# Potato256/my-mitsuba

Measured on AMD Instinct MI355X. Metric: Msamples/sec at 1280x720x256spp, 1/2/4/8 MI355X; per-pixel L1 vs CPU ref, higher is better.
Workload: dtype f32; 1 GPU; C3 bunny x15, 1,041,765 triangles, roughconductor Cu GGX 0.2, 15 instances flattened to world-space triangles; resolution=1280x720, spp=256, max_depth=8, parallelism=film tiles round-robin over 1 GPU(s), kd_build=host, kd_refs=4723933, kd_stop_prims=4

## Files before the change

include/mtsg.h:

```cpp
#ifndef MTSG_H
#define MTSG_H

#include <stdint.h>
#include <stddef.h>

#ifdef __cplusplus
extern "C" {
#endif

#define MTSG_ABI_VERSION 8

enum {
    MTSG_OK             = 0,
    MTSG_ERR_INVALID    = -1,
    MTSG_ERR_DEVICE     = -2,
    MTSG_ERR_OOM        = -3,
    MTSG_ERR_CANCELLED  = -4,
    MTSG_ERR_NODEVICE   = -5,
    MTSG_ERR_TRAVERSAL  = -6
};


typedef struct mtsg_kdnode {
    uint32_t combined;
// ... 349 lines not shown

int  mtsg_device_alloc(mtsg_scene *scene, size_t bytes, void **out);
int  mtsg_device_free(mtsg_scene *scene, void *ptr);
int  mtsg_device_memset(mtsg_scene *scene, void *ptr, size_t bytes);
int  mtsg_device_to_host(mtsg_scene *scene, void *dst, const void *src, size_t bytes);

void mtsg_cancel(mtsg_scene *scene);

void mtsg_cancel_clear(mtsg_scene *scene);

typedef void (*mtsg_tile_fn)(void *user, int32_t key, int32_t x, int32_t y, int32_t w, int32_t h);
int  mtsg_set_tile_callback(mtsg_scene *scene, mtsg_tile_fn fn, void *user);

int  mtsg_set_flags(mtsg_scene *scene, uint32_t flags);
int  mtsg_get_stats(mtsg_scene *scene, mtsg_stats *out);
int  mtsg_debug_wavetimes(mtsg_scene *scene, uint64_t *out, uint32_t max_launches, uint32_t *waves);
int  mtsg_debug_stragglers(mtsg_scene *scene, float *out, uint32_t max_rays);

int  mtsg_set_batch_paths(mtsg_scene *scene, uint32_t paths);

#define MTSG_DEFAULT_FINISH_PATHS 524288u
int  mtsg_set_finish_paths(mtsg_scene *scene, uint32_t paths);

#define MTSG_RECT_SETUP_CAP 2u
enum {
    MTSG_OPT_TRACE_REFILL = 1,
    MTSG_OPT_FINISH_SHADE_MIN = 2,
    MTSG_OPT_LANES = 3,
    MTSG_OPT_STAGGER = 4,
    MTSG_OPT_SHADE_GENERIC = 5,
    MTSG_OPT_RAY_ORDER = 6,
    MTSG_OPT_CAMERA_DIFFS = 7,
    MTSG_OPT_RECT_SETUP = 8,
    MTSG_OPT_RAY_PRESETUP = 9
};
int  mtsg_set_option(mtsg_scene *scene, int32_t key, int64_t value);

enum { MTSG_EMITTER_SET_AREA = 0, MTSG_EMITTER_SET_ENVMAP = 1, MTSG_EMITTER_SET_ALL = 2 };
int  mtsg_scene_kernel_sets(mtsg_scene *scene, int32_t *material_set, int32_t *emitter_set);

typedef struct mtsg_test_knobs {
    int32_t stack_cap, restart_guard, restart_limit, limit_shadow_only;
    int32_t no_instance_prefilter;
} mtsg_test_knobs;
int  mtsg_set_test_knobs(mtsg_scene *scene, const mtsg_test_knobs *knobs);

int  mtsg_env_eval(mtsg_scene *scene, uint32_t n, const float *dirs, const float *rx, const float *ry, float *out);

int  mtsg_tex_eval(mtsg_scene *scene, int tex, uint32_t n, const float *uv, const float *duv, float *out);

enum { MTSG_BSDF_QUERY_SAMPLE = 0, MTSG_BSDF_QUERY_EVAL = 1 };
enum { MTSG_BSDF_QUERY_OK = 1, MTSG_BSDF_QUERY_DELTA = 2, MTSG_BSDF_QUERY_NULL = 4 };
int  mtsg_bsdf_query(mtsg_scene *scene, int32_t bsdf, int32_t mode, uint32_t n, const float *in, const float *alb, float *out,
                     uint32_t *flags);

int  mtsg_om_query(mtsg_scene *scene, uint32_t n, const float *dirs, const float *o1, const float *o2, int32_t *ids,
                   int32_t *vis);
// ... 103 lines not shown
```

my-mitsuba_amd/csrc/kernels.h:

```cpp
#pragma once
#include <hip/hip_runtime.h>

#include <stdint.h>

#include "../../include/mtsg.h"
#include "device_math.h"
#include "envmap.h"
#include "sampler.h"

namespace mtsg {

struct DevCamera;
struct DevScene {
    const uint4 *__restrict__ blocks;
    uint2 root2;
    const float4 *__restrict__ triL;
    const float4 *__restrict__ vpos;
    const float4 *__restrict__ vnrm;
    const uint4 *__restrict__ tidx;
    const float4 *__restrict__ shrec;
    const mtsg_rect *__restrict__ rects;
    const float4 *__restrict__ rectM;
    uint32_t n_rect;
    const float4 *__restrict__ rectSh;
// ... 115 lines not shown
template <int SMP> void launch_finish_ext2(const ShadeLaunch &a);
#define MTSG_DECLARE_LAUNCHERS(SMP) \
    template <> void launch_shade_smp<SMP>(const ShadeLaunch &a); \
    template <> void launch_finish_smp<SMP>(const ShadeLaunch &a); \
    template <> void launch_shade_ext2<SMP>(const ShadeLaunch &a); \
    template <> void launch_finish_ext2<SMP>(const ShadeLaunch &a);
MTSG_DECLARE_LAUNCHERS(MTSG_SAMPLER_INDEPENDENT)
MTSG_DECLARE_LAUNCHERS(MTSG_SAMPLER_HALTON)
MTSG_DECLARE_LAUNCHERS(MTSG_SAMPLER_HAMMERSLEY)
MTSG_DECLARE_LAUNCHERS(MTSG_SAMPLER_LDSAMPLER)
MTSG_DECLARE_LAUNCHERS(MTSG_SAMPLER_SOBOL)
int finish_blocks_per_cu(bool mats);
struct FlatTraceLaunch {
    dim3 grid, tieGrid;
    hipStream_t stream;
    const DevScene *S;
    const DevPaths *P;
    int cIn, sIn;
    uint32_t n;
    unsigned long long *wt;
    bool count, knobs, refill32, tie;
    bool rectSetup;
    bool pre = false;
};
void launch_trace_flat(const FlatTraceLaunch &a);
int trace_flat_blocks_per_cu();

struct DevAov {
    int m;
    int pathChild;
    int nf;
    int kind[MTSG_MAX_SUBINTEGRATORS];
    int child[MTSG_MAX_SUBINTEGRATORS];
    float undef[MTSG_MAX_SUBINTEGRATORS][3];
    float w2c[16];
    const mtsg_aov_bsdf *bsdfs;
    const mtsg_aov_shape *shapes;
    const uint32_t *elems;
    float *planes;
    size_t cap;
};
struct FieldsLaunch {
    hipStream_t stream;
    const DevScene *S;
    const DevCamera *C;
    const DevIntegrator *I;
// ... 3769 lines not shown
```

my-mitsuba_amd/csrc/mtsg.hip:

```cpp
#include <hip/hip_runtime.h>

#include <algorithm>
#include <atomic>
#include <cstdio>
#include <cstdlib>
#include <cstring>
#include <mutex>
#include <string>
#include <unordered_map>
#include <vector>
#include <chrono>
#include <functional>

#include "../../include/mtsg.h"
#include "device_math.h"
#include "envmap.h"
#include "sampler.h"

#include "kernels.h"
#include "render_plan.h"

#ifndef MTSG_RAY_PRESETUP
#define MTSG_RAY_PRESETUP 0
#endif

static_assert(PLAN_TILE == TILE, "render_plan.h plans in tiles of kernels.h's edge");

namespace {

thread_local std::string g_err;

#define HIP_TRY(expr)                                                                  \
    do {                                                                               \
        hipError_t _e = (expr);                                                        \
        if (_e != hipSuccess) {                                                        \
            g_err = std::string(#expr) + ": " + hipGetErrorString(_e);                 \
            return _e == hipErrorOutOfMemory ? MTSG_ERR_OOM : MTSG_ERR_DEVICE;         \
        }                                                                              \
    } while (0)

template <class T>
int upload(const T *src, size_t n, T **dst) {
    *dst = nullptr;
    if (n == 0) return MTSG_OK;
    HIP_TRY(hipMalloc((void **)dst, n * sizeof(T)));
    HIP_TRY(hipMemcpy(*dst, src, n * sizeof(T), hipMemcpyHostToDevice));
// ... 33 lines not shown
    int lanesAlloc = 0;
    hipStream_t lstream[MTSG_MAX_LANES] = {};
    std::vector<int32_t> tileKeys;
    int32_t *tileKeysDev = nullptr;
    size_t tileKeysCap = 0;
    DevPaths LP[MTSG_MAX_LANES]{};
    std::vector<void *> batchAllocs;
    uint32_t *hostCnt = nullptr;
    int cuCount = 0;
    int traceGrid = 0, shadeGrid = 0, traceGridInst = 0, finishGrid = 0, finishGridMats = 0;
    uint32_t finishPaths = 0;
    uint32_t finishShadeMin = 16;
    uint32_t flags = 0;
    int samplerType = MTSG_SAMPLER_INDEPENDENT, samplerDim = 4;
    int qmcInv[2][3] = {{0, 0, 0}, {0, 0, 0}};
    int traceMode = 0;
    bool texDiffs = false, hasEnvmap = false, storeCamDiffs = false;
    int rayOrder = 0;
    float *dumpL = nullptr;
    std::atomic<int> cancel{0};
    bool knobs = false;
    bool rectSetupOpt = true, rectSetupOk = false;
    bool rayPresetupOpt = MTSG_RAY_PRESETUP != 0;
    mtsg_stats stats{};
    std::vector<hipEvent_t> evPool;
    size_t evUsed = 0;
    std::vector<std::pair<int, size_t>> timed;
    std::vector<unsigned long long> stragglers;
    unsigned long long *waveTimes = nullptr;
    uint32_t wtLaunches = 0;
    bool extBsdfs = false;
    bool ext2 = false;
    int mats = MATS_ALL;
    bool shadeGeneric = false;
    int emitterSet = EM_AREA;
    uint32_t nTextures = 0;
    const uint32_t *sobolM = nullptr;
    const uint64_t *sobolVdc = nullptr, *sobolVdcInv = nullptr;
    uint64_t sobolScramble = 0;
    bool aovOn = false;
    DevAov aov{};
    std::vector<void *> aovAllocs;
    float *fieldPlanes = nullptr;
    size_t fieldCap = 0;
    int fieldCount = 0;
    uint32_t nShapes = 0;
// ... 115 lines not shown
    return s->evPool[s->evUsed++];
}

template <class F>
void timed_launch(mtsg_scene *s, int kind, hipStream_t st, F f) {
    if (!(s->flags & MTSG_FLAG_TIMING)) { f(); return; }
    size_t i0 = s->evUsed;
    hipEventRecord(next_event(s), st);
    f();
    hipEventRecord(next_event(s), st);
    s->timed.emplace_back(kind, i0);
}

template <bool COUNT>
void launch_trace_c(mtsg_scene *s, const DevPaths &P, int cIn, int sIn, uint32_t n, hipStream_t st, bool pre) {
    dim3 g(s->traceGrid), blk(TRACE_BLOCK);
    unsigned long long *wt = nullptr;
    if ((s->flags & MTSG_FLAG_WAVETIME) && s->waveTimes && s->wtLaunches < WT_MAX_LAUNCHES && !s->ds.inst)
        wt = s->waveTimes + (size_t)WT_WORDS * s->traceGrid * s->wtLaunches++;
    const dim3 tg(std::max<unsigned>(1u, (unsigned)s->traceGrid / 4u));
    if (!s->ds.inst) {
        FlatTraceLaunch a{g, tg, st, &s->ds, &P, cIn, sIn, n, wt, COUNT, s->knobs, s->traceMode == 1,
                          MTSG_MAILBOX && cIn != -2 && !TIE_INLINE, s->rectSetupOpt && s->rectSetupOk, pre};
        launch_trace_flat(a);
        return;
    }
    if (s->knobs && !COUNT)
        hipLaunchKernelGGL((k_trace_s<false, MTSG_INST_MIN_IDLE, true, true>), dim3(s->traceGridInst), blk, 0, st, s->ds, P, cIn, sIn, n, wt);
    else hipLaunchKernelGGL((k_trace_s<COUNT, MTSG_INST_MIN_IDLE, true>), dim3(s->traceGridInst), blk, 0, st, s->ds, P, cIn, sIn, n, wt);
    if (MTSG_MAILBOX && cIn != -2) hipLaunchKernelGGL(k_tie_i, tg, blk, 0, st, s->ds, P);
}
void launch_trace(mtsg_scene *s, bool count, const DevPaths &P, int cIn, int sIn, uint32_t n, hipStream_t st, bool pre = false) {
    if (count) launch_trace_c<true>(s, P, cIn, sIn, n, st, pre);
    else launch_trace_c<false>(s, P, cIn, sIn, n, st, pre);
}
bool presetup_applies(const mtsg_scene *s) {
    return s->rayPresetupOpt && s->rectSetupOpt && s->rectSetupOk && !s->ds.inst && !s->knobs;
}

ShadeLaunch shade_args(mtsg_scene *s, const DevIntegrator &I, const DevBatch &B, const DevPaths &P, int b, int qin, hipStream_t st,
                       dim3 grid, dim3 block) {
    ShadeLaunch a;
    a.grid = grid;
    a.block = block;
    a.stream = st;
    a.S = &s->ds;
// ... 746 lines not shown
        if (ti.x >= d->n_vertices || ti.y >= d->n_vertices || ti.z >= d->n_vertices || ti.w >= d->n_shapes) {
            g_err = "triangle index out of range";
            return fail(MTSG_ERR_INVALID);
        }
        const float *P = d->vtx_pos, *N = d->vtx_nrm;
        float f[24];
        for (int k = 0; k < 3; ++k) {
            f[k] = P[3 * ti.x + k]; f[3 + k] = P[3 * ti.y + k]; f[6 + k] = P[3 * ti.z + k];
            f[9 + k] = N[3 * ti.x + k]; f[12 + k] = N[3 * ti.y + k]; f[15 + k] = N[3 * ti.z + k];
            f[18 + k] = d->tri_dpdu[3 * t + k];
        }
        const mtsg_shape &sh = d->shapes[ti.w];
        uint32_t u[3] = {ti.w, (uint32_t)sh.bsdf | (sh.face_normals ? 0x80000000u : 0u), (uint32_t)sh.emitter};
        memcpy(f + 21, u, sizeof(u));
        memcpy(&shrec[6 * (size_t)t], f, sizeof(f));
    }
    int rc;
    DevScene &ds = s->ds;
    auto up = [&](auto *src, size_t n, auto **dst) {
        int r = upload(src, n, dst);
        if (r == MTSG_OK && *dst) s->allocs.push_back((void *)*dst);
        return r;
    };
    std::vector<uint4> pairs;
    std::vector<float4> triL;
    pairs.reserve(d->n_nodes / 2 + 1);
    triL.reserve((size_t)d->n_indices * 3);
    bool layoutOk = true;
    const mtsg_kdnode *tNodes = d->nodes;
    const uint32_t *tIdx = d->indices;
    uint32_t tNodeCount = d->n_nodes, tIdxCount = d->n_indices;
    std::function<uint2(uint32_t, int)> convert = [&](uint32_t ni, int depth) -> uint2 {
        if (depth > 64 || ni >= tNodeCount) { layoutOk = false; return make_uint2(0x80000000u, 0u); }
        const mtsg_kdnode &N = tNodes[ni];
        if (N.combined & 0x80000000u) {
            const uint32_t start = (uint32_t)(triL.size() / 3);
            for (uint32_t e = N.combined & 0x7FFFFFFFu; e < N.data; ++e) {
                const uint32_t p = e < tIdxCount ? tIdx[e] : 0xFFFFFFFFu;
                if (p >= d->n_prims) { layoutOk = false; break; }
                mtsg_triaccel ta = d->triaccel[p];
                if (ta.k == MTSG_TRIACCEL_SHAPE && ta.shape_index < d->n_shapes &&
                    d->shapes[ta.shape_index].type == MTSG_SHAPE_INSTANCE) {
                    if (ta.prim_index >= d->n_instances) { layoutOk = false; break; }
                    ta.k = KINST;
                    const mtsg_instance &I = d->instances[ta.prim_index];
                    if (I.group >= d->n_groups) { layoutOk = false; break; }
                    const mtsg_group &G = d->groups[I.group];
                    double lo[3] = {INFINITY, INFINITY, INFINITY}, hi[3] = {-INFINITY, -INFINITY, -INFINITY};
                    for (int c = 0; c < 8; ++c) {
                        const double q[3] = {(c & 1) ? G.aabb_max[0] : G.aabb_min[0], (c & 2) ? G.aabb_max[1] : G.aabb_min[1],
                                             (c & 4) ? G.aabb_max[2] : G.aabb_min[2]};
                        for (int a = 0; a < 3; ++a) {
                            const float *W = I.to_world + 4 * a;
                            const double w = (double)W[0] * q[0] + (double)W[1] * q[1] + (double)W[2] * q[2] + (double)W[3];
                            lo[a] = std::min(lo[a], w);
                            hi[a] = std::max(hi[a], w);
                        }
                    }
                    double ext = 0, mag = 0;
                    for (int a = 0; a < 3; ++a) {
                        ext = std::max(ext, hi[a] - lo[a]);
                        mag = std::max(mag, std::max(std::fabs(lo[a]), std::fabs(hi[a])));
                    }
                    const double m = 1e-4 * (ext + mag) + 1e-30;
                    float bmin[3], bmax[3];
                    for (int a = 0; a < 3; ++a) {
                        bmin[a] = std::nextafter((float)(lo[a] - m), -INFINITY);
                        bmax[a] = std::nextafter((float)(hi[a] + m), INFINITY);
                    }
                    if (!std::isfinite(bmin[0] + bmin[1] + bmin[2] + bmax[0] + bmax[1] + bmax[2])) {
                        for (int a = 0; a < 3; ++a) { bmin[a] = -INFINITY; bmax[a] = INFINITY; }
                    }
                    ta.n_u = bmin[0]; ta.n_v = bmin[1]; ta.n_d = bmin[2];
                    ta.a_u = bmax[0]; ta.a_v = bmax[1]; ta.b_nu = bmax[2];
                }
                ta.shape_index = p;
                const float4 *t = (const float4 *)&ta;
                triL.push_back(t[0]); triL.push_back(t[1]); triL.push_back(t[2]);
            }
            return make_uint2(0x80000000u | start, (uint32_t)(triL.size() / 3));
        }
        const uint32_t left = ni + ((N.combined & ~(3u | 0x40000000u)) >> 2);
        const uint32_t pi = (uint32_t)pairs.size();
        pairs.push_back(make_uint4(0, 0, 0, 0));
        const uint2 L = convert(left, depth + 1);
        const uint2 R = convert(left + 1, depth + 1);
        pairs[pi] = make_uint4(L.x, L.y, R.x, R.y);
        return make_uint2((N.combined & 3u) | (pi << 2), N.data);
    };
    const uint2 root = convert(0, 0);
    std::vector<uint2> groupRoots(d->n_groups);
    if (d->n_instances && (!d->instances || !d->groups || !d->group_nodes || !d->group_indices)) layoutOk = false;
    for (uint32_t g = 0; g < d->n_groups && layoutOk; ++g) {
        const mtsg_group &G = d->groups[g];
        if ((uint64_t)G.node_offset + G.n_nodes > d->n_group_nodes || (uint64_t)G.index_offset + G.n_indices > d->n_group_indices ||
            G.n_nodes == 0) { layoutOk = false; break; }
        tNodes = d->group_nodes + G.node_offset;
        tIdx = d->group_indices + G.index_offset;
        tNodeCount = G.n_nodes;
        tIdxCount = G.n_indices;
        groupRoots[g] = convert(0, 0);
    }
    for (uint32_t i = 0; i < d->n_instances && layoutOk; ++i)
        if (d->instances[i].group >= d->n_groups) layoutOk = false;
    if (!layoutOk || pairs.size() >= (1u << 29) || triL.size() / 3 >= (1u << 30)) {
        g_err = "malformed or oversized kd-tree";
        return fail(MTSG_ERR_INVALID);
    }
    std::vector<uint4> blocks;
    blocks.reserve(pairs.size() * 2 + 8);
    std::unordered_map<uint32_t, uint32_t> preBlock;
    auto reserveBlock = [&](uint32_t pair) {
        preBlock[pair] = (uint32_t)(blocks.size() / 4);
        blocks.resize(blocks.size() + 4, make_uint4(0, 0, 0, 0));
    };
    if (!(root.x & 0x80000000u)) {
        reserveBlock(root.x >> 2);
        const uint4 pr = pairs[root.x >> 2];
        for (const uint2 c : {make_uint2(pr.x, pr.y), make_uint2(pr.z, pr.w)}) {
            if (c.x & 0x80000000u) continue;
            const uint4 gp = pairs[c.x >> 2];
            for (const uint2 g : {make_uint2(gp.x, gp.y), make_uint2(gp.z, gp.w)})
                if (!(g.x & 0x80000000u)) reserveBlock(g.x >> 2);
        }
    }
    std::function<uint2(uint2, bool, uint32_t)> conv2 = [&](uint2 w, bool root, uint32_t slot) -> uint2 {
        if (w.x & 0x80000000u) return w;
        const uint4 pr = pairs[w.x >> 2];
        const uint2 L = make_uint2(pr.x, pr.y), R = make_uint2(pr.z, pr.w);
        if (root) {
            uint32_t b;
            const auto pre = preBlock.find(w.x >> 2);
            if (pre != preBlock.end()) {
                b = pre->second;
            } else {
                b = (uint32_t)(blocks.size() / 4);
                blocks.resize(blocks.size() + 4, make_uint4(0, 0, 0, 0));
            }
            const uint2 nL = conv2(L, false, 4 * b + 1);
            const uint2 nR = conv2(R, false, 4 * b + 2);
            blocks[4 * b] = make_uint4(nL.x, nL.y, nR.x, nR.y);
            return make_uint2((w.x & 3u) | (b << 3), w.y);
        }
        const uint2 nL = conv2(L, true, 0), nR = conv2(R, true, 0);
        blocks[slot] = make_uint4(nL.x, nL.y, nR.x, nR.y);
        return make_uint2((w.x & 3u) | 4u | (slot << 3), w.y);
    };
    const uint2 root2 = conv2(root, true, 0);
    for (auto &gr : groupRoots) gr = conv2(gr, true, 0);
    blocks.resize(blocks.size() + 4, make_uint4(0, 0, 0, 0));
    if (blocks.size() < 20) blocks.resize(20, make_uint4(0, 0, 0, 0));
    if (blocks.size() >= (1u << 29)) { g_err = "kd-tree too large for the two-level layout"; return fail(MTSG_ERR_INVALID); }
    if (triL.empty()) triL.resize(3, make_float4(0, 0, 0, 0));
    uint4 *dblocks; float4 *dtriL; float4 *dvpos, *dvnrm, *dshrec; uint4 *dtidx;
    mtsg_rect *rects; mtsg_shape *shapes; mtsg_bsdf *bsdfs; mtsg_emitter *emitters; float *ecdf, *etcdf;
    if ((rc = up(triL.data(), triL.size(), &dtriL)) ||
        (rc = up(blocks.data(), blocks.size(), &dblocks)) ||
        (rc = up(vpos.data(), vpos.size(), &dvpos)) || (rc = up(vnrm.data(), vnrm.size(), &dvnrm)) ||
        (rc = up(tidx.data(), tidx.size(), &dtidx)) ||
        (rc = up(shrec.data(), shrec.size(), &dshrec)) ||
        (rc = up(d->rects, d->n_rects, &rects)) || (rc = up(d->shapes, d->n_shapes, &shapes)) ||
        (rc = up(d->bsdfs, d->n_bsdfs, &bsdfs)) || (rc = up(d->emitters, d->n_emitters, &emitters)) ||
        (rc = up(d->emitter_cdf, d->n_emitters + 1, &ecdf)) ||
        (rc = up(d->emitter_tri_cdf, d->n_emitter_tri_cdf, &etcdf)))
        return fail(rc);
    ds.blocks = dblocks; ds.root2 = root2;
    ds.triL = dtriL; ds.vpos = dvpos; ds.vnrm = dvnrm;
    int constantEmitter = -1;
    {
        std::vector<float4> rm((size_t)3 * std::max<uint32_t>(d->n_rects, 1u), make_float4(0, 0, 0, 0));
        for (uint32_t i = 0; i < d->n_rects; ++i)
            for (int k = 0; k < 3; ++k) {
                const float *m = d->rects[i].to_object + 4 * k;
                rm[3 * i + k] = make_float4(m[0], m[1], m[2], m[3]);
            }
        if (d->n_bsdfs >= 0xFFFFu || d->n_emitters >= 0xFFFEu) { g_err = "too many BSDFs or emitters"; return fail(MTSG_ERR_INVALID); }
        std::vector<float4> rs((size_t)2 * std::max<uint32_t>(d->n_rects, 1u), make_float4(0, 0, 0, 0));
        for (uint32_t i = 0; i < d->n_rects; ++i) {
            const mtsg_rect &R = d->rects[i];
            if (R.shape_index >= d->n_shapes) { g_err = "rectangle with an invalid shape index"; return fail(MTSG_ERR_INVALID); }
            const mtsg_shape &sh = d->shapes[R.shape_index];
            uint32_t be = ((uint32_t)sh.bsdf & 0xFFFFu) | (uint32_t)(sh.emitter + 1) << 16, si = R.shape_index;
            float bef, sif;
            memcpy(&bef, &be, 4);
            memcpy(&sif, &si, 4);
            rs[2 * i] = make_float4(R.frame_n[0], R.frame_n[1], R.frame_n[2], sif);
            rs[2 * i + 1] = make_float4(R.dpdu[0], R.dpdu[1], R.dpdu[2], bef);
        }
        std::vector<float4> er((size_t)4 * std::max<uint32_t>(d->n_emitters, 1u), make_float4(0, 0, 0, 0));
// ... 57 lines not shown
            memcpy(&er[4 * e + 3].w, &type, 4);
        }
        float4 *drm, *drs, *der;
        if ((rc = up(rm.data(), rm.size(), &drm)) || (rc = up(rs.data(), rs.size(), &drs)) || (rc = up(er.data(), er.size(), &der)))
            return fail(rc);
        ds.rectM = drm;
        ds.rectSh = drs;
        ds.emitRect = der;
    }
    ds.tidx = dtidx; ds.shrec = dshrec; ds.rects = rects; ds.shapes = shapes; ds.bsdfs = bsdfs;
    ds.emitters = emitters; ds.emitter_cdf = ecdf; ds.emitter_tri_cdf = etcdf;
    ds.inst = nullptr;
    if (d->n_instances) {
        std::vector<float4> in((size_t)8 * d->n_instances);
        for (uint32_t i = 0; i < d->n_instances; ++i) {
            const mtsg_instance &I = d->instances[i];
            const mtsg_group &G = d->groups[I.group];
            const float *L = I.to_local, *W = I.to_world;
            float4 *o = &in[8 * (size_t)i];
            for (int r = 0; r < 3; ++r) {
                o[r] = make_float4(L[4 * r], L[4 * r + 1], L[4 * r + 2], L[4 * r + 3]);
                o[3 + r] = make_float4(W[4 * r], W[4 * r + 1], W[4 * r + 2], W[4 * r + 3]);
            }
            const uint2 gr = groupRoots[I.group];
            float r0, r1;
            memcpy(&r0, &gr.x, 4);
            memcpy(&r1, &gr.y, 4);
            o[6] = make_float4(G.aabb_min[0], G.aabb_min[1], G.aabb_min[2], r0);
            o[7] = make_float4(G.aabb_max[0], G.aabb_max[1], G.aabb_max[2], r1);
        }
        float4 *dinst;
        if ((rc = up(in.data(), in.size(), &dinst))) return fail(rc);
        ds.inst = dinst;
    }
    ds.capFlat = SHORT_STACK;
    ds.capGrp = INNER_STACK;
    ds.capTop = OUTER_STACK;
    ds.rstGuard = RST_GUARD;
    ds.rstMax = RST_MAX;
    ds.rstMaxC = RST_MAX;
    ds.instPrefilter = 1;
    s->knobs = false;
    ds.instKeyStride = (uint64_t)d->n_prims * ((uint64_t)d->n_instances + 1) <= 0xFFFFFFFFull ? d->n_prims : 0x9E3779B1u;
    ds.has_env = d->has_envmap ? 1 : constantEmitter >= 0 ? 2 * (constantEmitter + 1) : 0;
    if (s->emitterSet != EM_ALL) s->emitterSet = d->has_envmap ? EM_ENV : EM_AREA;
    s->mats = 0;
    for (uint32_t i = 0; i < d->n_bsdfs; ++i) {
// ... 86 lines not shown
            tt[3 * t + 2] = make_float4(dv[2], 0.f, 0.f, 0.f);
        }
        float4 *dttex;
        if ((rc = up(tt.data(), tt.size(), &dttex))) return fail(rc);
        ds.ttex = dttex;
    }
    s->nShapes = d->n_shapes;
    s->bsdfTexture.resize(d->n_bsdfs);
    for (uint32_t i = 0; i < d->n_bsdfs; ++i) s->bsdfTexture[i] = d->bsdfs[i].texture;
    s->texDiffs = texDiffs;
    s->hasEnvmap = d->has_envmap != 0;
    ds.om = nullptr; ds.om_bits = nullptr;
    if (d->om) {
        if (!d->om_bits) { g_err = "occupancy maps without their bits"; return fail(MTSG_ERR_INVALID); }
        mtsg_om *dom; uint32_t *dbits;
        if ((rc = up(d->om, 1, &dom)) ||
            (rc = up(d->om_bits, (size_t)MTSG_OM_COUNT * MTSG_OM_SIZE * MTSG_OM_SIZE * (MTSG_OM_SIZE / 32), &dbits)))
            return fail(rc);
        ds.om = dom; ds.om_bits = dbits;
    }
    ds.n_emitters = d->n_emitters;
    ds.n_tri = d->n_triangles;
    ds.n_rect = d->n_rects;
    s->rectSetupOk = MTSG_RECT_SETUP && d->n_rects <= RECT_SETUP_CAP;
    for (uint32_t r = 0; r < d->n_rects && s->rectSetupOk; ++r) {
        const mtsg_triaccel &ta = d->triaccel[d->n_triangles + r];
        s->rectSetupOk = ta.k == MTSG_TRIACCEL_SHAPE && ta.prim_index == r && ta.shape_index < d->n_shapes &&
                         d->shapes[ta.shape_index].type == MTSG_SHAPE_RECT;
    }
    ds.n_bsdfs = d->n_bsdfs;
    for (int k = 0; k < 3; ++k) { ds.bmin[k] = d->aabb_min[k]; ds.bmax[k] = d->aabb_max[k]; }
    DevCamera &c = s->cam;
    const mtsg_camera &hc = d->camera;
    memcpy(c.s2c, hc.sample_to_camera, sizeof(c.s2c));
    memcpy(c.c2w, hc.camera_to_world, sizeof(c.c2w));
    c.near_clip = hc.near_clip; c.far_clip = hc.far_clip; c.inv_res_x = hc.inv_res_x; c.inv_res_y = hc.inv_res_y;
    c.film_w = hc.film_w; c.film_h = hc.film_h;
    c.filter_radius = hc.filter_radius; c.filter_scale = hc.filter_scale; c.border = hc.border;
    c.has_alpha = hc.has_alpha;
    memcpy(c.filter_values, hc.filter_values, sizeof(c.filter_values));
    memcpy(c.dx, hc.dx, sizeof(c.dx));
    memcpy(c.dy, hc.dy, sizeof(c.dy));
    c.crop_w = hc.crop_w; c.crop_h = hc.crop_h;
    c.lens = hc.sensor_type == MTSG_SENSOR_THINLENS ? 1 : 0;
    c.aperture_radius = hc.aperture_radius; c.focus_distance = hc.focus_distance;
    ds.camO[0] = c.c2w[3]; ds.camO[1] = c.c2w[7]; ds.camO[2] = c.c2w[11];
    ds.camNear = c.near_clip; ds.camFar = c.far_clip;
    ds.camCompact = (ds.inst || c.lens) ? 0 : 1;
    c.compact = ds.camCompact;
    camera_diff_mode(s);
    {
        DevCamera *dc;
// ... 140 lines not shown
            if (value < 0 || value > 16) { g_err = "MTSG_OPT_STAGGER: 0..16 bounces"; return MTSG_ERR_INVALID; }
            s->stagger = (int)value;
            return MTSG_OK;
        case MTSG_OPT_SHADE_GENERIC:
            s->shadeGeneric = value != 0;
            return MTSG_OK;
        case MTSG_OPT_RAY_ORDER:
            if (value < 0 || value > 1) { g_err = "MTSG_OPT_RAY_ORDER: 0 (append order) or 1 (direction-sorted windows)"; return MTSG_ERR_INVALID; }
            s->rayOrder = (int)value;
            return MTSG_OK;
        case MTSG_OPT_CAMERA_DIFFS:
            if (value < 0 || value > 1) { g_err = "MTSG_OPT_CAMERA_DIFFS: 0 (recomputed on a miss) or 1 (stored)"; return MTSG_ERR_INVALID; }
            s->storeCamDiffs = value != 0;
            camera_diff_mode(s);
            return MTSG_OK;
        case MTSG_OPT_RECT_SETUP:
            if (value < 0 || value > 1) { g_err = "MTSG_OPT_RECT_SETUP: 0 (rectangles tested in the leaves) or 1 (at ray setup)"; return MTSG_ERR_INVALID; }
            s->rectSetupOpt = value != 0;
            return MTSG_OK;
        case MTSG_OPT_RAY_PRESETUP:
            if (value < 0 || value > 1) { g_err = "MTSG_OPT_RAY_PRESETUP: 0 (rectangles tested in the traversal's refill) or 1 (where the rays are made)"; return MTSG_ERR_INVALID; }
            s->rayPresetupOpt = value != 0;
            return MTSG_OK;
        default:
            g_err = "unknown option key " + std::to_string(key);
            return MTSG_ERR_INVALID;
    }
}

int mtsg_set_flags(mtsg_scene *s, uint32_t flags) {
    if (!s) return MTSG_ERR_INVALID;
    s->flags = flags;
    return MTSG_OK;
}

int mtsg_get_stats(mtsg_scene *s, mtsg_stats *out) {
    if (!s || !out) return MTSG_ERR_INVALID;
    *out = s->stats;
    return MTSG_OK;
}

int mtsg_debug_wavetimes(mtsg_scene *s, uint64_t *out, uint32_t max_launches, uint32_t *waves) {
    if (!s || !waves || (!out && max_launches)) return MTSG_ERR_INVALID;
    *waves = (uint32_t)s->traceGrid;
    const uint32_t n = std::min(max_launches, s->wtLaunches);
    if (n && s->waveTimes &&
// ... 649 lines not shown
```

my-mitsuba_amd/csrc/trace_flat.hip:

```cpp
#pragma clang diagnostic ignored "-Wunused-function"
#ifndef MTSG_STACK_LANE
#define MTSG_STACK_LANE 1
#endif
#include "kernels.h"

#if MTSG_FLAT_REGS
namespace {
#define FLAT_TRACE_KERNEL(MIN_IDLE, KNOBS)                                                                               \
    template <>                                                                                                          \
    __global__ void FLAT_TRACE_ATTR k_trace_s<false, MIN_IDLE, false, KNOBS>(DevScene S, DevPaths P, int cIn, int sIn,   \
                                                                             uint32_t nIdentity, unsigned long long *wt) { \
        trace_s_body<false, MIN_IDLE, false, KNOBS>(S, P, cIn, sIn, nIdentity, wt);                                      \
    }
FLAT_TRACE_KERNEL(16, false)
FLAT_TRACE_KERNEL(32, false)
FLAT_TRACE_KERNEL(16, true)
#undef FLAT_TRACE_KERNEL
}
#endif

namespace mtsg {

template <bool COUNT>
static void launch_flat(const FlatTraceLaunch &a) {
    const dim3 blk(TRACE_BLOCK);
    if (a.pre && a.rectSetup && !a.knobs) {
        if (a.refill32) hipLaunchKernelGGL((k_trace_s_pre<COUNT, 32>), a.grid, blk, 0, a.stream, *a.S, *a.P, a.cIn, a.sIn, a.n, a.wt);
        else hipLaunchKernelGGL((k_trace_s_pre<COUNT, 16>), a.grid, blk, 0, a.stream, *a.S, *a.P, a.cIn, a.sIn, a.n, a.wt);
    } else if (a.knobs && !COUNT) hipLaunchKernelGGL((k_trace_s<false, 16, false, true>), a.grid, blk, 0, a.stream, *a.S, *a.P, a.cIn, a.sIn, a.n, a.wt);
    else if (!a.rectSetup && a.refill32) hipLaunchKernelGGL((k_trace_s_leaf<COUNT, 32>), a.grid, blk, 0, a.stream, *a.S, *a.P, a.cIn, a.sIn, a.n, a.wt);
    else if (!a.rectSetup) hipLaunchKernelGGL((k_trace_s_leaf<COUNT, 16>), a.grid, blk, 0, a.stream, *a.S, *a.P, a.cIn, a.sIn, a.n, a.wt);
    else if (a.refill32) hipLaunchKernelGGL((k_trace_s<COUNT, 32>), a.grid, blk, 0, a.stream, *a.S, *a.P, a.cIn, a.sIn, a.n, a.wt);
    else hipLaunchKernelGGL((k_trace_s<COUNT, 16>), a.grid, blk, 0, a.stream, *a.S, *a.P, a.cIn, a.sIn, a.n, a.wt);
    if (a.tie) {
        if (a.knobs) hipLaunchKernelGGL((k_tie<true>), a.tieGrid, blk, 0, a.stream, *a.S, *a.P);
        else hipLaunchKernelGGL((k_tie<false>), a.tieGrid, blk, 0, a.stream, *a.S, *a.P);
    }
}

void launch_trace_flat(const FlatTraceLaunch &a) {
    if (a.count) launch_flat<true>(a);
    else launch_flat<false>(a);
}

int trace_flat_blocks_per_cu() {
    int perCU = 0;
    if (hipOccupancyMaxActiveBlocksPerMultiprocessor(&perCU, (const void *)k_trace_s<false, 16>, TRACE_BLOCK, 0) != hipSuccess) return 0;
    return perCU;
}
// ... 3 lines not shown
```

my-mitsuba_amd/mtsg.py:

```python
from __future__ import annotations

import ctypes as C
import os

import numpy as np

PKG_DIR = os.path.dirname(os.path.abspath(__file__))
REPO_DIR = os.path.dirname(PKG_DIR)

MTSG_OK = 0
MTSH_INSTANCING_FLATTEN = 0
MTSH_INSTANCING_TWO_LEVEL = 1
MTSG_FLAG_TIMING = 1
MTSG_FLAG_COUNT = 2
MTSG_FLAG_WAVETIME = 4
MTSG_OPT_TRACE_REFILL = 1
MTSG_OPT_FINISH_SHADE_MIN = 2
MTSG_OPT_LANES = 3
MTSG_OPT_STAGGER = 4
MTSG_OPT_SHADE_GENERIC = 5
MTSG_OPT_RAY_ORDER = 6
MTSG_OPT_CAMERA_DIFFS = 7
MTSG_OPT_RECT_SETUP = 8
MTSG_OPT_RAY_PRESETUP = 9
MTSG_RECT_SETUP_CAP = 2
MTSG_INTEGRATOR_PATH = 0
MTSG_INTEGRATOR_PATH2_OM = 1
MTSG_INTEGRATOR_DIRECT = 2
MTSG_INTEGRATOR_AO = 3
MTSG_EMITTER_AREA, MTSG_EMITTER_ENVMAP, MTSG_EMITTER_POINT, MTSG_EMITTER_SPOT = 1, 2, 3, 4
MTSG_EMITTER_DIRECTIONAL, MTSG_EMITTER_CONSTANT = 5, 6


class RenderParams(C.Structure):
    _fields_ = [
        ("max_depth", C.c_int32), ("rr_depth", C.c_int32),
        ("strict_normals", C.c_int32), ("hide_emitters", C.c_int32),
        ("spp", C.c_uint32), ("seed", C.c_uint32),
        ("tile_x", C.c_int32), ("tile_y", C.c_int32),
        ("tile_w", C.c_int32), ("tile_h", C.c_int32),
        ("tile_stride", C.c_int32), ("tile_offset", C.c_int32),
        ("integrator", C.c_int32), ("om_strategy", C.c_int32), ("om_mis", C.c_int32), ("om_jitter", C.c_int32),
    ]

    def copy(self) -> "RenderParams":
        p = RenderParams()
        C.memmove(C.byref(p), C.byref(self), C.sizeof(RenderParams))
        return p
# ... 1093 lines not shown
```

Baseline: 1813 Msamples/s.

## Build rect-free kd leaf copies for the rect-setup trace path

```diff
diff --git a/include/mtsg.h b/include/mtsg.h
--- a/include/mtsg.h
+++ b/include/mtsg.h
@@ -395,7 +395,7 @@
 #define MTSG_DEFAULT_FINISH_PATHS 524288u
 int  mtsg_set_finish_paths(mtsg_scene *scene, uint32_t paths);
 
-#define MTSG_RECT_SETUP_CAP 2u
+#define MTSG_RECT_SETUP_CAP 8u
 enum {
     MTSG_OPT_TRACE_REFILL = 1,
     MTSG_OPT_FINISH_SHADE_MIN = 2,
@@ -405,7 +405,8 @@
     MTSG_OPT_RAY_ORDER = 6,
     MTSG_OPT_CAMERA_DIFFS = 7,
     MTSG_OPT_RECT_SETUP = 8,
-    MTSG_OPT_RAY_PRESETUP = 9
+    MTSG_OPT_RAY_PRESETUP = 9,
+    MTSG_OPT_LEAF_FILTER = 10
 };
 int  mtsg_set_option(mtsg_scene *scene, int32_t key, int64_t value);
 
diff --git a/my-mitsuba_amd/csrc/kd_layout.h b/my-mitsuba_amd/csrc/kd_layout.h
--- /dev/null
+++ b/my-mitsuba_amd/csrc/kd_layout.h
@@ -0,0 +1,218 @@
+#pragma once
+
+#include <algorithm>
+#include <cmath>
+#include <cstdint>
+#include <cstring>
+#include <functional>
+#include <unordered_map>
+#include <vector>
+
+#include "../../include/mtsg.h"
+
+namespace mtsg {
+
+struct KdU2 { uint32_t x, y; };
+struct KdU4 { uint32_t x, y, z, w; };
+struct KdF4 { float x, y, z, w; };
+static_assert(sizeof(KdU4) == 16 && sizeof(KdF4) == 16 && sizeof(mtsg_triaccel) == 48, "uploaded as uint4 / float4 / 3 float4");
+
+constexpr uint32_t KD_KINST = 4u;
+
+struct KdLayout {
+    std::vector<KdU4> blocks;
+    std::vector<KdF4> triL;
+    KdU2 root2{};
+    std::vector<KdU2> groupRoots;
+    std::vector<KdU4> blocksRS;
+    KdU2 root2RS{};
+    size_t triBase = 0;
+    size_t leavesFiltered = 0, leavesEmptied = 0;
+};
+
+inline const char *kd_layout(const mtsg_scene_desc *d, bool filter, KdLayout &out) {
+    auto u2 = [](uint32_t x, uint32_t y) { return KdU2{x, y}; };
+    auto u4 = [](uint32_t x, uint32_t y, uint32_t z, uint32_t w) { return KdU4{x, y, z, w}; };
+    std::vector<KdU4> pairs;
+    std::vector<KdF4> &triL = out.triL;
+    triL.clear();
+    pairs.reserve(d->n_nodes / 2 + 1);
+    triL.reserve((size_t)d->n_indices * 3);
+    bool layoutOk = true;
+    const mtsg_kdnode *tNodes = d->nodes;
+    const uint32_t *tIdx = d->indices;
+    uint32_t tNodeCount = d->n_nodes, tIdxCount = d->n_indices;
+    filter = filter && d->n_groups == 0 && d->n_instances == 0;
+    std::vector<KdU2> rectLeaves;
+    std::function<KdU2(uint32_t, int)> convert = [&](uint32_t ni, int depth) -> KdU2 {
+        if (depth > 64 || ni >= tNodeCount) { layoutOk = false; return u2(0x80000000u, 0u); }
+        const mtsg_kdnode &N = tNodes[ni];
+        if (N.combined & 0x80000000u) {
+            const uint32_t start = (uint32_t)(triL.size() / 3);
+            bool hasRect = false;
+            for (uint32_t e = N.combined & 0x7FFFFFFFu; e < N.data; ++e) {
+                const uint32_t p = e < tIdxCount ? tIdx[e] : 0xFFFFFFFFu;
+                if (p >= d->n_prims) { layoutOk = false; break; }
+                mtsg_triaccel ta = d->triaccel[p];
+                if (ta.k == MTSG_TRIACCEL_SHAPE && ta.shape_index < d->n_shapes &&
+                    d->shapes[ta.shape_index].type == MTSG_SHAPE_INSTANCE) {
+                    if (ta.prim_index >= d->n_instances) { layoutOk = false; break; }
+                    ta.k = KD_KINST;
+                    const mtsg_instance &I = d->instances[ta.prim_index];
+                    if (I.group >= d->n_groups) { layoutOk = false; break; }
+                    const mtsg_group &G = d->groups[I.group];
+                    double lo[3] = {INFINITY, INFINITY, INFINITY}, hi[3] = {-INFINITY, -INFINITY, -INFINITY};
+                    for (int c = 0; c < 8; ++c) {
+                        const double q[3] = {(c & 1) ? G.aabb_max[0] : G.aabb_min[0], (c & 2) ? G.aabb_max[1] : G.aabb_min[1],
+                                             (c & 4) ? G.aabb_max[2] : G.aabb_min[2]};
+                        for (int a = 0; a < 3; ++a) {
+                            const float *W = I.to_world + 4 * a;
+                            const double w = (double)W[0] * q[0] + (double)W[1] * q[1] + (double)W[2] * q[2] + (double)W[3];
+                            lo[a] = std::min(lo[a], w);
+                            hi[a] = std::max(hi[a], w);
+                        }
+                    }
+                    double ext = 0, mag = 0;
+                    for (int a = 0; a < 3; ++a) {
+                        ext = std::max(ext, hi[a] - lo[a]);
+                        mag = std::max(mag, std::max(std::fabs(lo[a]), std::fabs(hi[a])));
+                    }
+                    const double m = 1e-4 * (ext + mag) + 1e-30;
+                    float bmin[3], bmax[3];
+                    for (int a = 0; a < 3; ++a) {
+                        bmin[a] = std::nextafter((float)(lo[a] - m), -INFINITY);
+                        bmax[a] = std::nextafter((float)(hi[a] + m), INFINITY);
+                    }
+                    if (!std::isfinite(bmin[0] + bmin[1] + bmin[2] + bmax[0] + bmax[1] + bmax[2])) {
+                        for (int a = 0; a < 3; ++a) { bmin[a] = -INFINITY; bmax[a] = INFINITY; }
+                    }
+                    ta.n_u = bmin[0]; ta.n_v = bmin[1]; ta.n_d = bmin[2];
+                    ta.a_u = bmax[0]; ta.a_v = bmax[1]; ta.b_nu = bmax[2];
+                }
+                hasRect |= ta.k == MTSG_TRIACCEL_SHAPE;
+                ta.shape_index = p;
+                KdF4 t[3];
+                memcpy(t, &ta, sizeof(t));
+                triL.push_back(t[0]); triL.push_back(t[1]); triL.push_back(t[2]);
+            }
+            const KdU2 w = u2(0x80000000u | start, (uint32_t)(triL.size() / 3));
+            if (filter && hasRect) rectLeaves.push_back(w);
+            return w;
+        }
+        const uint32_t left = ni + ((N.combined & ~(3u | 0x40000000u)) >> 2);
+        const uint32_t pi = (uint32_t)pairs.size();
+        pairs.push_back(u4(0, 0, 0, 0));
+        const KdU2 L = convert(left, depth + 1);
+        const KdU2 R = convert(left + 1, depth + 1);
+        pairs[pi] = u4(L.x, L.y, R.x, R.y);
+        return u2((N.combined & 3u) | (pi << 2), N.data);
+    };
+    const KdU2 root = convert(0, 0);
+    std::vector<KdU2> &groupRoots = out.groupRoots;
+    groupRoots.assign(d->n_groups, u2(0, 0));
+    if (d->n_instances && (!d->instances || !d->groups || !d->group_nodes || !d->group_indices)) layoutOk = false;
+    for (uint32_t g = 0; g < d->n_groups && layoutOk; ++g) {
+        const mtsg_group &G = d->groups[g];
+        if ((uint64_t)G.node_offset + G.n_nodes > d->n_group_nodes || (uint64_t)G.index_offset + G.n_indices > d->n_group_indices ||
+            G.n_nodes == 0) { layoutOk = false; break; }
+        tNodes = d->group_nodes + G.node_offset;
+        tIdx = d->group_indices + G.index_offset;
+        tNodeCount = G.n_nodes;
+        tIdxCount = G.n_indices;
+        groupRoots[g] = convert(0, 0);
+    }
+    for (uint32_t i = 0; i < d->n_instances && layoutOk; ++i)
+        if (d->instances[i].group >= d->n_groups) layoutOk = false;
+    if (!layoutOk || pairs.size() >= (1u << 29) || triL.size() / 3 >= (1u << 30)) return "malformed or oversized kd-tree";
+    std::vector<KdU4> &blocks = out.blocks;
+    blocks.clear();
+    blocks.reserve(pairs.size() * 2 + 8);
+    std::unordered_map<uint32_t, uint32_t> preBlock;
+    auto reserveBlock = [&](uint32_t pair) {
+        preBlock[pair] = (uint32_t)(blocks.size() / 4);
+        blocks.resize(blocks.size() + 4, u4(0, 0, 0, 0));
+    };
+    if (!(root.x & 0x80000000u)) {
+        reserveBlock(root.x >> 2);
+        const KdU4 pr = pairs[root.x >> 2];
+        for (const KdU2 c : {u2(pr.x, pr.y), u2(pr.z, pr.w)}) {
+            if (c.x & 0x80000000u) continue;
+            const KdU4 gp = pairs[c.x >> 2];
+            for (const KdU2 g : {u2(gp.x, gp.y), u2(gp.z, gp.w)})
+                if (!(g.x & 0x80000000u)) reserveBlock(g.x >> 2);
+        }
+    }
+    std::vector<uint64_t> leafSlots;
+    auto noteLeaves = [&](size_t slot, KdU2 l, KdU2 r) {
+        if (!filter) return;
+        if (l.x & 0x80000000u) leafSlots.push_back(2 * (uint64_t)slot);
+        if (r.x & 0x80000000u) leafSlots.push_back(2 * (uint64_t)slot + 1);
+    };
+    std::function<KdU2(KdU2, bool, uint32_t)> conv2 = [&](KdU2 w, bool isRoot, uint32_t slot) -> KdU2 {
+        if (w.x & 0x80000000u) return w;
+        const KdU4 pr = pairs[w.x >> 2];
+        const KdU2 L = u2(pr.x, pr.y), R = u2(pr.z, pr.w);
+        if (isRoot) {
+            uint32_t b;
+            const auto pre = preBlock.find(w.x >> 2);
+            if (pre != preBlock.end()) {
+                b = pre->second;
+            } else {
+                b = (uint32_t)(blocks.size() / 4);
+                blocks.resize(blocks.size() + 4, u4(0, 0, 0, 0));
+            }
+            const KdU2 nL = conv2(L, false, 4 * b + 1);
+            const KdU2 nR = conv2(R, false, 4 * b + 2);
+            blocks[4 * b] = u4(nL.x, nL.y, nR.x, nR.y);
+            noteLeaves(4 * (size_t)b, nL, nR);
+            return u2((w.x & 3u) | (b << 3), w.y);
+        }
+        const KdU2 nL = conv2(L, true, 0), nR = conv2(R, true, 0);
+        blocks[slot] = u4(nL.x, nL.y, nR.x, nR.y);
+        noteLeaves(slot, nL, nR);
+        return u2((w.x & 3u) | 4u | (slot << 3), w.y);
+    };
+    out.root2 = conv2(root, true, 0);
+    for (auto &gr : groupRoots) gr = conv2(gr, true, 0);
+    blocks.resize(blocks.size() + 4, u4(0, 0, 0, 0));
+    if (blocks.size() < 20) blocks.resize(20, u4(0, 0, 0, 0));
+    if (blocks.size() >= (1u << 29)) return "kd-tree too large for the two-level layout";
+    out.triBase = triL.size() / 3;
+    out.blocksRS.clear();
+    out.root2RS = out.root2;
+    out.leavesFiltered = out.leavesEmptied = 0;
+    if (!rectLeaves.empty()) {
+        std::unordered_map<uint32_t, KdU2> moved;
+        moved.reserve(rectLeaves.size() * 2);
+        for (const KdU2 w : rectLeaves) {
+            const uint32_t st = (uint32_t)(triL.size() / 3);
+            for (uint32_t e = w.x & 0x7FFFFFFFu; e < w.y; ++e) {
+                uint32_t k;
+                memcpy(&k, &triL[3 * (size_t)e].x, 4);
+                if (k == MTSG_TRIACCEL_SHAPE) continue;
+                for (int j = 0; j < 3; ++j) { const KdF4 f = triL[3 * (size_t)e + j]; triL.push_back(f); }
+            }
+            const uint32_t en = (uint32_t)(triL.size() / 3);
+            moved[w.x] = st < en ? u2(0x80000000u | st, en) : u2(w.x, w.x & 0x7FFFFFFFu);
+            ++out.leavesFiltered;
+            out.leavesEmptied += st == en;
+        }
+        if (triL.size() / 3 >= (1u << 30)) return "kd-tree too large for the filtered leaf records";
+        auto remap = [&](KdU2 w) {
+            if (!(w.x & 0x80000000u) || (w.x & 0x7FFFFFFFu) >= w.y) return w;
+            const auto it = moved.find(w.x);
+            return it == moved.end() ? w : it->second;
+        };
+        out.blocksRS = blocks;
+        for (const uint64_t s : leafSlots) {
+            KdU4 &b = out.blocksRS[(size_t)(s >> 1)];
+            if (s & 1) { const KdU2 n = remap(u2(b.z, b.w)); b.z = n.x; b.w = n.y; }
+            else { const KdU2 n = remap(u2(b.x, b.y)); b.x = n.x; b.y = n.y; }
+        }
+        out.root2RS = remap(out.root2);
+    }
+    if (triL.empty()) triL.resize(3, KdF4{0, 0, 0, 0});
+    return nullptr;
+}
+
+}
diff --git a/my-mitsuba_amd/csrc/kernels.h b/my-mitsuba_amd/csrc/kernels.h
--- a/my-mitsuba_amd/csrc/kernels.h
+++ b/my-mitsuba_amd/csrc/kernels.h
@@ -161,6 +161,9 @@
     bool count, knobs, refill32, tie;
     bool rectSetup;
     bool pre = false;
+    bool leafFilter = false;
+    const uint4 *blocksRS = nullptr;
+    uint2 root2RS = {0u, 0u};
 };
 void launch_trace_flat(const FlatTraceLaunch &a);
 int trace_flat_blocks_per_cu();
diff --git a/my-mitsuba_amd/csrc/mtsg.hip b/my-mitsuba_amd/csrc/mtsg.hip
--- a/my-mitsuba_amd/csrc/mtsg.hip
+++ b/my-mitsuba_amd/csrc/mtsg.hip
@@ -19,9 +19,13 @@
 
 #include "kernels.h"
 #include "render_plan.h"
+#include "kd_layout.h"
 
 #ifndef MTSG_RAY_PRESETUP
 #define MTSG_RAY_PRESETUP 0
+#endif
+#ifndef MTSG_LEAF_FILTER
+#define MTSG_LEAF_FILTER 1
 #endif
 
 static_assert(PLAN_TILE == TILE, "render_plan.h plans in tiles of kernels.h's edge");
@@ -101,6 +105,9 @@
     bool knobs = false;
     bool rectSetupOpt = true, rectSetupOk = false;
     bool rayPresetupOpt = MTSG_RAY_PRESETUP != 0;
+    bool leafFilterOpt = MTSG_LEAF_FILTER != 0;
+    const uint4 *blocksRS = nullptr;
+    uint2 root2RS{};
     mtsg_stats stats{};
     std::vector<hipEvent_t> evPool;
     size_t evUsed = 0;
@@ -262,6 +269,9 @@
     if (!s->ds.inst) {
         FlatTraceLaunch a{g, tg, st, &s->ds, &P, cIn, sIn, n, wt, COUNT, s->knobs, s->traceMode == 1,
                           MTSG_MAILBOX && cIn != -2 && !TIE_INLINE, s->rectSetupOpt && s->rectSetupOk, pre};
+        a.leafFilter = s->leafFilterOpt && s->blocksRS != nullptr;
+        a.blocksRS = s->blocksRS;
+        a.root2RS = s->root2RS;
         launch_trace_flat(a);
         return;
     }
@@ -1054,140 +1064,26 @@
         if (r == MTSG_OK && *dst) s->allocs.push_back((void *)*dst);
         return r;
     };
-    std::vector<uint4> pairs;
-    std::vector<float4> triL;
-    pairs.reserve(d->n_nodes / 2 + 1);
-    triL.reserve((size_t)d->n_indices * 3);
-    bool layoutOk = true;
-    const mtsg_kdnode *tNodes = d->nodes;
-    const uint32_t *tIdx = d->indices;
-    uint32_t tNodeCount = d->n_nodes, tIdxCount = d->n_indices;
-    std::function<uint2(uint32_t, int)> convert = [&](uint32_t ni, int depth) -> uint2 {
-        if (depth > 64 || ni >= tNodeCount) { layoutOk = false; return make_uint2(0x80000000u, 0u); }
-        const mtsg_kdnode &N = tNodes[ni];
-        if (N.combined & 0x80000000u) {
-            const uint32_t start = (uint32_t)(triL.size() / 3);
-            for (uint32_t e = N.combined & 0x7FFFFFFFu; e < N.data; ++e) {
-                const uint32_t p = e < tIdxCount ? tIdx[e] : 0xFFFFFFFFu;
-                if (p >= d->n_prims) { layoutOk = false; break; }
-                mtsg_triaccel ta = d->triaccel[p];
-                if (ta.k == MTSG_TRIACCEL_SHAPE && ta.shape_index < d->n_shapes &&
-                    d->shapes[ta.shape_index].type == MTSG_SHAPE_INSTANCE) {
-                    if (ta.prim_index >= d->n_instances) { layoutOk = false; break; }
-                    ta.k = KINST;
-                    const mtsg_instance &I = d->instances[ta.prim_index];
-                    if (I.group >= d->n_groups) { layoutOk = false; break; }
-                    const mtsg_group &G = d->groups[I.group];
-                    double lo[3] = {INFINITY, INFINITY, INFINITY}, hi[3] = {-INFINITY, -INFINITY, -INFINITY};
-                    for (int c = 0; c < 8; ++c) {
-                        const double q[3] = {(c & 1) ? G.aabb_max[0] : G.aabb_min[0], (c & 2) ? G.aabb_max[1] : G.aabb_min[1],
-                                             (c & 4) ? G.aabb_max[2] : G.aabb_min[2]};
-                        for (int a = 0; a < 3; ++a) {
-                            const float *W = I.to_world + 4 * a;
-                            const double w = (double)W[0] * q[0] + (double)W[1] * q[1] + (double)W[2] * q[2] + (double)W[3];
-                            lo[a] = std::min(lo[a], w);
-                            hi[a] = std::max(hi[a], w);
-                        }
-                    }
-                    double ext = 0, mag = 0;
-                    for (int a = 0; a < 3; ++a) {
-                        ext = std::max(ext, hi[a] - lo[a]);
-                        mag = std::max(mag, std::max(std::fabs(lo[a]), std::fabs(hi[a])));
-                    }
-                    const double m = 1e-4 * (ext + mag) + 1e-30;
-                    float bmin[3], bmax[3];
-                    for (int a = 0; a < 3; ++a) {
-                        bmin[a] = std::nextafter((float)(lo[a] - m), -INFINITY);
-                        bmax[a] = std::nextafter((float)(hi[a] + m), INFINITY);
-                    }
-                    if (!std::isfinite(bmin[0] + bmin[1] + bmin[2] + bmax[0] + bmax[1] + bmax[2])) {
-                        for (int a = 0; a < 3; ++a) { bmin[a] = -INFINITY; bmax[a] = INFINITY; }
-                    }
-                    ta.n_u = bmin[0]; ta.n_v = bmin[1]; ta.n_d = bmin[2];
-                    ta.a_u = bmax[0]; ta.a_v = bmax[1]; ta.b_nu = bmax[2];
-                }
-                ta.shape_index = p;
-                const float4 *t = (const float4 *)&ta;
-                triL.push_back(t[0]); triL.push_back(t[1]); triL.push_back(t[2]);
-            }
-            return make_uint2(0x80000000u | start, (uint32_t)(triL.size() / 3));
-        }
-        const uint32_t left = ni + ((N.combined & ~(3u | 0x40000000u)) >> 2);
-        const uint32_t pi = (uint32_t)pairs.size();
-        pairs.push_back(make_uint4(0, 0, 0, 0));
-        const uint2 L = convert(left, depth + 1);
-        const uint2 R = convert(left + 1, depth + 1);
-        pairs[pi] = make_uint4(L.x, L.y, R.x, R.y);
-        return make_uint2((N.combined & 3u) | (pi << 2), N.data);
-    };
-    const uint2 root = convert(0, 0);
-    std::vector<uint2> groupRoots(d->n_groups);
-    if (d->n_instances && (!d->instances || !d->groups || !d->group_nodes || !d->group_indices)) layoutOk = false;
-    for (uint32_t g = 0; g < d->n_groups && layoutOk; ++g) {
-        const mtsg_group &G = d->groups[g];
-        if ((uint64_t)G.node_offset + G.n_nodes > d->n_group_nodes || (uint64_t)G.index_offset + G.n_indices > d->n_group_indices ||
-            G.n_nodes == 0) { layoutOk = false; break; }
-        tNodes = d->group_nodes + G.node_offset;
-        tIdx = d->group_indices + G.index_offset;
-        tNodeCount = G.n_nodes;
-        tIdxCount = G.n_indices;
-        groupRoots[g] = convert(0, 0);
-    }
-    for (uint32_t i = 0; i < d->n_instances && layoutOk; ++i)
-        if (d->instances[i].group >= d->n_groups) layoutOk = false;
-    if (!layoutOk || pairs.size() >= (1u << 29) || triL.size() / 3 >= (1u << 30)) {
-        g_err = "malformed or oversized kd-tree";
+    s->rectSetupOk = MTSG_RECT_SETUP && d->n_rects <= RECT_SETUP_CAP;
+    for (uint32_t r = 0; r < d->n_rects && s->rectSetupOk; ++r) {
+        if (!d->triaccel || (uint64_t)d->n_triangles + r >= d->n_prims) { s->rectSetupOk = false; break; }
+        const mtsg_triaccel &ta = d->triaccel[d->n_triangles + r];
+        s->rectSetupOk = ta.k == MTSG_TRIACCEL_SHAPE && ta.prim_index == r && ta.shape_index < d->n_shapes &&
+                         d->shapes[ta.shape_index].type == MTSG_SHAPE_RECT;
+    }
+    KdLayout lay;
+    if (const char *what = kd_layout(d, s->rectSetupOk && d->n_rects > 0 && d->n_instances == 0, lay)) {
+        g_err = what;
         return fail(MTSG_ERR_INVALID);
     }
-    std::vector<uint4> blocks;
-    blocks.reserve(pairs.size() * 2 + 8);
-    std::unordered_map<uint32_t, uint32_t> preBlock;
-    auto reserveBlock = [&](uint32_t pair) {
-        preBlock[pair] = (uint32_t)(blocks.size() / 4);
-        blocks.resize(blocks.size() + 4, make_uint4(0, 0, 0, 0));
-    };
-    if (!(root.x & 0x80000000u)) {
-        reserveBlock(root.x >> 2);
-        const uint4 pr = pairs[root.x >> 2];
-        for (const uint2 c : {make_uint2(pr.x, pr.y), make_uint2(pr.z, pr.w)}) {
-            if (c.x & 0x80000000u) continue;
-            const uint4 gp = pairs[c.x >> 2];
-            for (const uint2 g : {make_uint2(gp.x, gp.y), make_uint2(gp.z, gp.w)})
-                if (!(g.x & 0x80000000u)) reserveBlock(g.x >> 2);
-        }
-    }
-    std::function<uint2(uint2, bool, uint32_t)> conv2 = [&](uint2 w, bool root, uint32_t slot) -> uint2 {
-        if (w.x & 0x80000000u) return w;
-        const uint4 pr = pairs[w.x >> 2];
-        const uint2 L = make_uint2(pr.x, pr.y), R = make_uint2(pr.z, pr.w);
-        if (root) {
-            uint32_t b;
-            const auto pre = preBlock.find(w.x >> 2);
-            if (pre != preBlock.end()) {
-                b = pre->second;
-            } else {
-                b = (uint32_t)(blocks.size() / 4);
-                blocks.resize(blocks.size() + 4, make_uint4(0, 0, 0, 0));
-            }
-            const uint2 nL = conv2(L, false, 4 * b + 1);
-            const uint2 nR = conv2(R, false, 4 * b + 2);
-            blocks[4 * b] = make_uint4(nL.x, nL.y, nR.x, nR.y);
-            return make_uint2((w.x & 3u) | (b << 3), w.y);
-        }
-        const uint2 nL = conv2(L, true, 0), nR = conv2(R, true, 0);
-        blocks[slot] = make_uint4(nL.x, nL.y, nR.x, nR.y);
-        return make_uint2((w.x & 3u) | 4u | (slot << 3), w.y);
-    };
-    const uint2 root2 = conv2(root, true, 0);
-    for (auto &gr : groupRoots) gr = conv2(gr, true, 0);
-    blocks.resize(blocks.size() + 4, make_uint4(0, 0, 0, 0));
-    if (blocks.size() < 20) blocks.resize(20, make_uint4(0, 0, 0, 0));
-    if (blocks.size() >= (1u << 29)) { g_err = "kd-tree too large for the two-level layout"; return fail(MTSG_ERR_INVALID); }
-    if (triL.empty()) triL.resize(3, make_float4(0, 0, 0, 0));
-    uint4 *dblocks; float4 *dtriL; float4 *dvpos, *dvnrm, *dshrec; uint4 *dtidx;
+    static_assert(sizeof(KdU4) == sizeof(uint4) && sizeof(KdF4) == sizeof(float4), "kd_layout.h arrays upload as uint4 / float4");
+    const std::vector<KdU2> &groupRoots = lay.groupRoots;
+    const uint2 root2 = make_uint2(lay.root2.x, lay.root2.y);
+    uint4 *dblocks, *dblocksRS; float4 *dtriL; float4 *dvpos, *dvnrm, *dshrec; uint4 *dtidx;
     mtsg_rect *rects; mtsg_shape *shapes; mtsg_bsdf *bsdfs; mtsg_emitter *emitters; float *ecdf, *etcdf;
-    if ((rc = up(triL.data(), triL.size(), &dtriL)) ||
-        (rc = up(blocks.data(), blocks.size(), &dblocks)) ||
+    if ((rc = up(reinterpret_cast<const float4 *>(lay.triL.data()), lay.triL.size(), &dtriL)) ||
+        (rc = up(reinterpret_cast<const uint4 *>(lay.blocks.data()), lay.blocks.size(), &dblocks)) ||
+        (rc = up(reinterpret_cast<const uint4 *>(lay.blocksRS.data()), lay.blocksRS.size(), &dblocksRS)) ||
         (rc = up(vpos.data(), vpos.size(), &dvpos)) || (rc = up(vnrm.data(), vnrm.size(), &dvnrm)) ||
         (rc = up(tidx.data(), tidx.size(), &dtidx)) ||
         (rc = up(shrec.data(), shrec.size(), &dshrec)) ||
@@ -1197,6 +1093,8 @@
         (rc = up(d->emitter_tri_cdf, d->n_emitter_tri_cdf, &etcdf)))
         return fail(rc);
     ds.blocks = dblocks; ds.root2 = root2;
+    s->blocksRS = dblocksRS;
+    s->root2RS = make_uint2(lay.root2RS.x, lay.root2RS.y);
     ds.triL = dtriL; ds.vpos = dvpos; ds.vnrm = dvnrm;
     int constantEmitter = -1;
     {
@@ -1300,7 +1198,7 @@
                 o[r] = make_float4(L[4 * r], L[4 * r + 1], L[4 * r + 2], L[4 * r + 3]);
                 o[3 + r] = make_float4(W[4 * r], W[4 * r + 1], W[4 * r + 2], W[4 * r + 3]);
             }
-            const uint2 gr = groupRoots[I.group];
+            const KdU2 gr = groupRoots[I.group];
             float r0, r1;
             memcpy(&r0, &gr.x, 4);
             memcpy(&r1, &gr.y, 4);
@@ -1433,12 +1331,6 @@
     ds.n_emitters = d->n_emitters;
     ds.n_tri = d->n_triangles;
     ds.n_rect = d->n_rects;
-    s->rectSetupOk = MTSG_RECT_SETUP && d->n_rects <= RECT_SETUP_CAP;
-    for (uint32_t r = 0; r < d->n_rects && s->rectSetupOk; ++r) {
-        const mtsg_triaccel &ta = d->triaccel[d->n_triangles + r];
-        s->rectSetupOk = ta.k == MTSG_TRIACCEL_SHAPE && ta.prim_index == r && ta.shape_index < d->n_shapes &&
-                         d->shapes[ta.shape_index].type == MTSG_SHAPE_RECT;
-    }
     ds.n_bsdfs = d->n_bsdfs;
     for (int k = 0; k < 3; ++k) { ds.bmin[k] = d->aabb_min[k]; ds.bmax[k] = d->aabb_max[k]; }
     DevCamera &c = s->cam;
@@ -1625,6 +1517,10 @@
             if (value < 0 || value > 1) { g_err = "MTSG_OPT_RAY_PRESETUP: 0 (rectangles tested in the traversal's refill) or 1 (where the rays are made)"; return MTSG_ERR_INVALID; }
             s->rayPresetupOpt = value != 0;
             return MTSG_OK;
+        case MTSG_OPT_LEAF_FILTER:
+            if (value < 0 || value > 1) { g_err = "MTSG_OPT_LEAF_FILTER: 0 (the setup mode steps over rectangle records) or 1 (its leaves hold none)"; return MTSG_ERR_INVALID; }
+            s->leafFilterOpt = value != 0;
+            return MTSG_OK;
         default:
             g_err = "unknown option key " + std::to_string(key);
             return MTSG_ERR_INVALID;
diff --git a/my-mitsuba_amd/csrc/trace_flat.hip b/my-mitsuba_amd/csrc/trace_flat.hip
--- a/my-mitsuba_amd/csrc/trace_flat.hip
+++ b/my-mitsuba_amd/csrc/trace_flat.hip
@@ -24,7 +24,15 @@
 template <bool COUNT>
 static void launch_flat(const FlatTraceLaunch &a) {
     const dim3 blk(TRACE_BLOCK);
-    if (a.pre && a.rectSetup && !a.knobs) {
+    if (!COUNT && a.leafFilter && a.blocksRS && a.rectSetup && !a.knobs) {
+        DevScene S = *a.S;
+        S.blocks = a.blocksRS;
+        S.root2 = a.root2RS;
+        if (a.pre && a.refill32) hipLaunchKernelGGL((k_trace_s_pre<COUNT, 32>), a.grid, blk, 0, a.stream, S, *a.P, a.cIn, a.sIn, a.n, a.wt);
+        else if (a.pre) hipLaunchKernelGGL((k_trace_s_pre<COUNT, 16>), a.grid, blk, 0, a.stream, S, *a.P, a.cIn, a.sIn, a.n, a.wt);
+        else if (a.refill32) hipLaunchKernelGGL((k_trace_s<COUNT, 32>), a.grid, blk, 0, a.stream, S, *a.P, a.cIn, a.sIn, a.n, a.wt);
+        else hipLaunchKernelGGL((k_trace_s<COUNT, 16>), a.grid, blk, 0, a.stream, S, *a.P, a.cIn, a.sIn, a.n, a.wt);
+    } else if (a.pre && a.rectSetup && !a.knobs) {
         if (a.refill32) hipLaunchKernelGGL((k_trace_s_pre<COUNT, 32>), a.grid, blk, 0, a.stream, *a.S, *a.P, a.cIn, a.sIn, a.n, a.wt);
         else hipLaunchKernelGGL((k_trace_s_pre<COUNT, 16>), a.grid, blk, 0, a.stream, *a.S, *a.P, a.cIn, a.sIn, a.n, a.wt);
     } else if (a.knobs && !COUNT) hipLaunchKernelGGL((k_trace_s<false, 16, false, true>), a.grid, blk, 0, a.stream, *a.S, *a.P, a.cIn, a.sIn, a.n, a.wt);
diff --git a/my-mitsuba_amd/mtsg.py b/my-mitsuba_amd/mtsg.py
--- a/my-mitsuba_amd/mtsg.py
+++ b/my-mitsuba_amd/mtsg.py
@@ -23,7 +23,8 @@
 MTSG_OPT_CAMERA_DIFFS = 7
 MTSG_OPT_RECT_SETUP = 8
 MTSG_OPT_RAY_PRESETUP = 9
-MTSG_RECT_SETUP_CAP = 2
+MTSG_OPT_LEAF_FILTER = 10
+MTSG_RECT_SETUP_CAP = 8
 MTSG_INTEGRATOR_PATH = 0
 MTSG_INTEGRATOR_PATH2_OM = 1
 MTSG_INTEGRATOR_DIRECT = 2
```

Result: faster. 1895 Msamples/s (median of 6 runs) (+4.5%).
